# apapiu/transformer_latent_diffusion

Measured on AMD Instinct MI355X. Metric: images/sec (256px, 35-step CFG sampling), denoiser only, higher is better.
Workload: dtype bf16; 1 GPU; C1: 100M-param denoiser (d=768, L=12), 32x32x4 latents, 35 steps + CFG 6, DPM-Solver++(2M), 64 images/GPU (model batch 128); images_per_gpu=64, global_batch=64, n_iter=35, parallelism=single GPU

## Files before the change

transformer_latent_diffusion_amd/csrc/tld_gemm.hip:

```cpp
#include "../../include/tld_hip.h"
#include "tld_common.h"
#include "tld_attn_core.h"
#include <cstdlib>
#include <cstring>
#include <type_traits>

#ifdef TLD_DBG_EPI
#define TLD_EPI_BIT(b) ((p.dbg_epi & (b)) != 0)
#else
#define TLD_EPI_BIT(b) false
#endif

namespace tld {

namespace {

typedef const __attribute__((address_space(1))) void* gptr_t;
typedef __attribute__((address_space(3))) void* lptr_t;

__device__ __forceinline__ bf16x8 read_frag(const char* lds_tile, int row, int kchunk) {
    const int off = row * 128 + ((kchunk ^ ((row >> 1) & 7)) << 4);
    return *reinterpret_cast<const bf16x8*>(lds_tile + off);
}

// ... 30 lines not shown
    static constexpr int CB2_OFF = ROWSTAT2_OFF + 256 * 8;
    static constexpr int UPDW2_LDS = CB2_OFF + 2048;
    static constexpr int PLAINRS_OFF = LDS_BYTES;
    static constexpr int PLAINCB_OFF = PLAINRS_OFF + 256 * 8;
    static constexpr int PLAINLN_LDS = PLAINCB_OFF + 2048;
    static constexpr int SCRATCH = 4608;
    static constexpr int AT_K = STAGE_BYTES, AT_V = AT_K + 256 * 128, AT_Q = AT_V + 64 * kAttnVPitch, ATTN_LDS = AT_Q + 256 * 128;
};

template <int BN, int EPI, bool F8 = false, bool CONV = false, bool RING = false, bool TN = false>
__global__ __launch_bounds__(512) void gemm256p_kernel(GemmParams p, int nblocks) {
    using G = G256P<BN>;
    static_assert(!RING || BN == 256, "the half-tile ring exists for 256 x 256 tiles (bf16, and since round 6 MX-fp8)");
    static_assert(!TN || (BN == 256 && EPI == EPI_F32 && !F8 && !CONV && !RING), "transposed operands: fp32 output, 256 x 256 tiles, two-stage loop");
    using frag_t = std::conditional_t<F8, i32x8, bf16x8>;
    constexpr int ESZ = F8 ? 1 : 2;
    constexpr int SC_OFF = G::LDS_BYTES;
    static_assert(!F8 || (EPI == EPI_F32 || EPI == EPI_QKV || EPI == EPI_BIAS_BF16 || EPI == EPI_BIAS_RESID), "fp8 epilogues");
    static_assert(!CONV || (!F8 && (EPI == EPI_F32 || EPI == EPI_BIAS_BF16 || EPI == EPI_BIAS_RESID)), "conv mode");
    constexpr bool PLAIN_CB = EPI == EPI_BIAS_BF16 && BN != 384 && !F8 && !CONV;
    constexpr bool IS_QKV = EPI == EPI_QKV || EPI == EPI_QKV_LN, LN = EPI == EPI_QKV_LN || EPI == EPI_QKV_ATTN;
    constexpr bool UPDW = EPI == EPI_UP_DWCONV2 || EPI == EPI_UP_DWCONV32;
    static_assert(EPI != EPI_QKV_ATTN || (BN == 192 && !F8 && !CONV && !RING), "the fused attention epilogue is written for 256 x 192 tiles");
    static_assert(EPI != EPI_QKV_ATTN || G::ATTN_LDS <= 160 * 1024, "LDS");
    static_assert(8 * G::SCRATCH <= G::STAGE_BYTES, "epilogue scratch must fit in one stage");
    extern __shared__ __attribute__((aligned(16))) char smem[];
    const int lane = threadIdx.x & 63;
    const int wid = __builtin_amdgcn_readfirstlane(threadIdx.x >> 6);
    const int wm = wid / G::WN, wn = wid % G::WN;
    const int l31 = lane & 31, hi = lane >> 5;

    const int ntn = (p.N + BN - 1) / BN;
    const int ntm = (p.M + G::BM - 1) / G::BM;
    constexpr bool KSPLIT_OK = EPI == EPI_F32 && !F8 && !CONV && !RING && !TN;
    const int nsplit = (KSPLIT_OK && p.ksplit > 1) ? p.ksplit : 1;
    const int ntiles = ntm * ntn * nsplit;
    int kb_dec = 0;
    const int bid = blockIdx.x;
    const int xcd = bid & 7, lidx = bid >> 3;
    const int per_xcd_blocks = (nblocks + 7 - xcd) / 8;
    const int G2 = p.xcd_ngroups > 1 ? p.xcd_ngroups : 1;
    const int xn = xcd % G2, xm = xcd / G2, XM = 8 / G2;
    const int gcols = ntn / G2;
    const int r0 = (int)((long)ntm * xm / XM), r1 = (int)((long)ntm * (xm + 1) / XM);
    const int q = ntiles >> 3, rr = ntiles & 7;
    const int xbase = xcd < rr ? xcd * (q + 1) : rr * (q + 1) + (xcd - rr) * q;
    const int xcount = G2 > 1 ? (r1 - r0) * gcols : q + (xcd < rr ? 1 : 0);
    int my_tiles = lidx < xcount ? (xcount - lidx + per_xcd_blocks - 1) / per_xcd_blocks : 0;
    constexpr bool HT_OK = RING && !CONV && (EPI == EPI_F32 || EPI == EPI_QKV || EPI == EPI_QKV_LN || EPI == EPI_BIAS_BF16);
    const int ht_q = xcount / per_xcd_blocks, ht_R = xcount - ht_q * per_xcd_blocks;
    const bool ht = HT_OK && p.half_tail && G2 == 1 && ht_R > 0 && 2 * ht_R <= per_xcd_blocks;
    const int ht_qa = lidx >= ht_R ? 1 : 0;
    if (ht) my_tiles = ht_q + (lidx < 2 * ht_R ? 1 : 0);
// ... 4 lines not shown
    auto tile_coords = [&](int i, int& m0, int& n0) {
        const int t = item_tile(i);
        if (G2 > 1) {
            const int tm = t / gcols;
            m0 = (r0 + tm) * G::BM;
            n0 = (xn * gcols + (t - tm * gcols)) * BN;
        } else {
            int tile = xbase + t;
            if constexpr (KSPLIT_OK) {
                if (nsplit > 1) {
                    const int sp = tile / (ntm * ntn);
                    tile -= sp * (ntm * ntn);
                    kb_dec = sp * p.K * 2;
                }
            }
            const int tm = tile / ntn;
            m0 = tm * G::BM;
            n0 = (tile - tm * ntn) * BN;
        }
    };
    if (my_tiles == 0) return;

    const int nk = CONV ? 9 * (p.cv_cin >> 6) : p.K * ESZ / (G::BK * 2);
    unsigned voffA[G::A_PIECES], voffB[G::B_PIECES];
    unsigned cpix[G::A_PIECES], cbase[G::A_PIECES];
    size_t tnA = 0, tnW = 0;
    auto conv_tap = [&](int tap) {
        if constexpr (CONV) {
            const int ky = tap / 3;
            const int dy = ky - 1 + p.cv_down, dx = tap - ky * 3 - 1 + p.cv_down;
            const int ws_ = (p.cv_w >> p.cv_up) << p.cv_down;
            const unsigned sh = (unsigned)(p.cv_h << p.cv_down), sw = (unsigned)(p.cv_w << p.cv_down);
            int ln = lane;
            asm volatile("" : "+v"(ln));
#pragma unroll
            for (int q2 = 0; q2 < G::A_PIECES; ++q2) {
                const int r = (wid * G::A_PIECES + q2) * 8 + (ln >> 3);
                const unsigned c16 = (unsigned)(((ln & 7) ^ ((r >> 1) & 7)) * 16);
                const int yy = (int)(cpix[q2] >> 16) + dy, xx = (int)(cpix[q2] & 0xffffu) + dx;
                const bool inb = (unsigned)yy < sh && (unsigned)xx < sw;
                const unsigned sp = cbase[q2] + (unsigned)((yy >> p.cv_up) * ws_ + (xx >> p.cv_up));
                unsigned v = inb ? p.cv_data_off + sp * (unsigned)(p.cv_cin * 2) + c16 : c16;
                asm volatile("" : "+v"(v));
                voffA[q2] = v;
            }
        }
    };
// ... 28 lines not shown
                gr = gr < p.M ? gr : p.M - 1;
                const unsigned b = (unsigned)gr / hw, rem = (unsigned)gr - b * hw;
                const unsigned y = rem / (unsigned)p.cv_w, x = rem - y * (unsigned)p.cv_w;
                cpix[q2] = ((y << 16) | x) << p.cv_down;
                cbase[q2] = b * shw;
            }
            conv_tap(0);
        } else {
#pragma unroll
        for (int q2 = 0; q2 < G::A_PIECES; ++q2) {
            const int r = (wid * G::A_PIECES + q2) * 8 + (ln >> 3);
            const int clog = (ln & 7) ^ ((r >> 1) & 7);
            int gr = tm0 + r;
            gr = gr < p.M ? gr : p.M - 1;
            unsigned v = __umul24((unsigned)gr, (unsigned)(p.lda * ESZ)) + (unsigned)(clog * 16);
            asm volatile("" : "+v"(v));
            voffA[q2] = v;
        }
        }
        unsigned wgrp = 0;
        if constexpr (!F8 && !CONV && (EPI == EPI_F32 || EPI == EPI_BIAS_BF16)) {
            if (p.w_batch_rows) wgrp = (unsigned)(tm0 / p.w_batch_rows) * p.w_batch_stride_bytes;
        }
#pragma unroll
        for (int q2 = 0; q2 < G::B_PIECES; ++q2) {
            const int r = (wid * G::B_PIECES + q2) * 8 + (ln >> 3);
            const int clog = (ln & 7) ^ ((r >> 1) & 7);
            int gr = tn0 + r;
            gr = gr < p.N ? gr : p.N - 1;
            unsigned v = __umul24((unsigned)gr, (unsigned)(p.ldw * ESZ)) + (unsigned)(clog * 16) + wgrp;
            asm volatile("" : "+v"(v));
            voffB[q2] = v;
        }
    };
    int conv_akb = 0;
    auto dma_piece = [&](int q2, int kbyte, char* st) {
        if constexpr (TN) {
            const bool isA = q2 < G::A_PIECES;
            const char* base = isA ? reinterpret_cast<const char*>(p.A) + tnA + (size_t)(kbyte >> 7) * 64 * p.lda * 2
                                   : reinterpret_cast<const char*>(p.W) + tnW + (size_t)(kbyte >> 7) * 64 * p.ldw * 2;
            const unsigned vo = isA ? voffA[q2] : voffB[q2 - G::A_PIECES];
            __builtin_amdgcn_global_load_lds((gptr_t)(base + vo), (lptr_t)(st + (isA ? 0 : G::A_BYTES) + (wid * G::A_PIECES + (isA ? q2 : q2 - G::A_PIECES)) * 1024), 16, 0, 0);
            return;
        }
        if (q2 < G::A_PIECES) {
            const char* base = reinterpret_cast<const char*>(p.A) + (CONV ? conv_akb : kbyte);
            __builtin_amdgcn_global_load_lds((gptr_t)(base + voffA[q2]), (lptr_t)(st + (wid * G::A_PIECES + q2) * 1024), 16, 0, 0);
        } else {
            const char* base = reinterpret_cast<const char*>(p.W) + kbyte;
            __builtin_amdgcn_global_load_lds((gptr_t)(base + voffB[q2 - G::A_PIECES]),
                                             (lptr_t)(st + G::A_BYTES + (wid * G::B_PIECES + (q2 - G::A_PIECES)) * 1024), 16, 0, 0);
        }
    };
    auto dma_scales = [&](int tm0, int tn0, int kstep, int stage) {
        if constexpr (F8) {
            if (wid < 2) {
                const int rows = wid == 0 ? p.M : p.N;
                int r = (wid == 0 ? tm0 : tn0) + lane * 4;
                r = r + 3 < rows ? r : rows - 4;
                const uint8_t* src = (wid == 0 ? p.a_scale : p.w_scale) + ((size_t)kstep * rows + r) * 4;
                __builtin_amdgcn_global_load_lds((gptr_t)src, (lptr_t)(smem + SC_OFF + stage * 2048 + wid * 1024), 16, 0, 0);
            }
        }
    };
    auto issue = [&](int m0, int n0, int g) {
        char* st = smem + (g & 1) * G::STAGE_BYTES;
        set_offsets(m0, n0);
#pragma unroll
        for (int q2 = 0; q2 < G::A_PIECES + G::B_PIECES; ++q2) dma_piece(q2, KSPLIT_OK ? kb_dec : 0, st);
        dma_scales(m0, n0, 0, g & 1);
// ... 20 lines not shown
#pragma unroll
            for (int i = 0; i < G::TM; ++i) a[i] = rd(tnoA[i]);
#pragma unroll
            for (int j = 0; j < G::TN; ++j) b[j] = rd(tnoB[j]);
        } else if constexpr (!F8) {
            const int kc = ks * 2 + hi;
#pragma unroll
            for (int i = 0; i < G::TM; ++i) a[i] = read_frag(st, wm * G::WROWS + i * 32 + l31, kc);
#pragma unroll
            for (int j = 0; j < G::TN; ++j) b[j] = read_frag(st + G::A_BYTES, wn * G::WCOLS + j * 32 + l31, kc);
        } else {
            const int c = ks * 4 + hi;
            auto rd = [&](const char* base, int row) {
                const int sw = (row >> 1) & 7;
                const u32x4 lo = *reinterpret_cast<const u32x4*>(base + row * 128 + ((c ^ sw) << 4));
                const u32x4 hi4 = *reinterpret_cast<const u32x4*>(base + row * 128 + (((c + 2) ^ sw) << 4));
                return i32x8{(int)lo[0], (int)lo[1], (int)lo[2], (int)lo[3], (int)hi4[0], (int)hi4[1], (int)hi4[2], (int)hi4[3]};
            };
#pragma unroll
            for (int i = 0; i < G::TM; ++i) a[i] = rd(st, wm * G::WROWS + i * 32 + l31);
#pragma unroll
            for (int j = 0; j < G::TN; ++j) b[j] = rd(st + G::A_BYTES, wn * G::WCOLS + j * 32 + l31);
        }
    };

    constexpr int HT = 16384;
    unsigned rvA[RING ? 4 : 1], rvB[RING ? 4 : 1];
    unsigned rcpix[RING && CONV ? 4 : 1], rcbase[RING && CONV ? 4 : 1];
    int sc_m0 = 0, sc_n0 = 0;
    auto ring_conv_tap = [&](int tap) {
        if constexpr (RING && CONV) {
            const int ky = tap / 3;
            const int dy = ky - 1 + p.cv_down, dx = tap - ky * 3 - 1 + p.cv_down;
            const int ws_ = (p.cv_w >> p.cv_up) << p.cv_down;
            const unsigned sh = (unsigned)(p.cv_h << p.cv_down), sw = (unsigned)(p.cv_w << p.cv_down);
            unsigned full = ~0u;
            asm volatile("" : "+s"(full));
            int ln = (int)__builtin_amdgcn_mbcnt_hi(full, __builtin_amdgcn_mbcnt_lo(full, 0u));
            asm volatile("" : "+v"(ln));
#pragma unroll
            for (int h = 0; h < 2; ++h)
#pragma unroll
                for (int q2 = 0; q2 < 2; ++q2) {
                    const int r = (wid * 2 + q2) * 8 + (ln >> 3);
                    const unsigned c16 = (unsigned)(((ln & 7) ^ ((r >> 1) & 7)) * 16);
                    const int yy = (int)(rcpix[h * 2 + q2] >> 16) + dy, xx = (int)(rcpix[h * 2 + q2] & 0xffffu) + dx;
// ... 91 lines not shown

    int m0, n0;
    tile_coords(0, m0, n0);
    int kb0 = kb_dec, kbn = 0;
    if constexpr (!RING) issue(m0, n0, 0);
    int g = 0;
    int ctap = 0, ccb = 0;
    const int kpt = CONV ? (p.cv_cin >> 6) : 1;
    for (int it = 0; it < my_tiles; ++it) {
        int m0n = 0, n0n = 0;
        const bool has_next = it + 1 < my_tiles;
        if (has_next) { tile_coords(it + 1, m0n, n0n); kbn = kb_dec; }
        constexpr bool swapped = EPI != EPI_F32 && !UPDW;
        bool v_tile = false;
        if constexpr (IS_QKV) v_tile = n0 >= 2 * p.d;

        int nkt = nk;
        if constexpr (TN) {
            const int split = p.w_batch_rows ? m0 / p.w_batch_rows : 0;
            const int rows = p.tn_ktotal - split * p.K;
            nkt = (rows < p.K ? rows : p.K) >> 6;
        }
        const bool hmode = ht && it == ht_q;
        f32x16 acc[G::TM][G::TN];
#pragma unroll
        for (int i = 0; i < G::TM; ++i)
#pragma unroll
            for (int j = 0; j < G::TN; ++j)
#pragma unroll
                for (int r = 0; r < 16; ++r) acc[i][j][r] = 0.f;

        frag_t a0[G::TM], b0[G::TN];
        int sca[G::TM], scb[G::TN];
        auto aux_dma = [&]() {
            if constexpr (LN) {
                static_assert(kLnSlots == 8, "one partial-sum row is 64 B");
#pragma unroll
                for (int q2 = 0; q2 < 2; ++q2) {
                    const int piece = wid * 2 + q2;
                    int row = m0 + piece * 16 + (lane >> 2);
                    row = row < p.M ? row : p.M - 1;
                    const char* src = reinterpret_cast<const char*>(p.ln_stats) + (size_t)row * 64 + (lane & 3) * 16;
                    __builtin_amdgcn_global_load_lds((gptr_t)src, (lptr_t)(smem + G::LN_RAW + piece * 1024), 16, 0, 0);
                }
                if (wid < 2) {
                    int col = n0 + lane * 4;
                    col = col < p.N ? col : 0;
                    const float* src = (wid == 0 ? p.ln_c1 : p.ln_b1) + col;
                    __builtin_amdgcn_global_load_lds((gptr_t)src, (lptr_t)(smem + G::LN_CB + wid * 1024), 16, 0, 0);
                }
            }
            if constexpr (EPI == EPI_BIAS_BF16) {
                if (BN != 384 && p.row_stats && wid < 2) {
                    int r0s = m0 + wid * 128 + lane * 2;
                    r0s = r0s + 1 < p.M ? r0s : (p.M >= 2 ? p.M - 2 : 0);
// ... 3 lines not shown
                if constexpr (PLAIN_CB) {
                    if (wid == 3 || (wid == 2 && p.row_stats)) {
                        int col = n0 + lane * 4;
                        col = col < p.N ? col : 0;
                        const float* src = (wid == 2 ? p.ln_c1 : p.bias) + col;
                        __builtin_amdgcn_global_load_lds((gptr_t)src, (lptr_t)(smem + G::PLAINCB_OFF + (wid - 2) * 1024), 16, 0, 0);
                    }
                }
            }
            if constexpr (UPDW) {
                constexpr int RS_OFF = G::ROWSTAT2_OFF;
                if (p.row_stats && wid < 2) {
                    const char* src = reinterpret_cast<const char*>(p.row_stats + m0) + wid * 1024 + lane * 16;
                    __builtin_amdgcn_global_load_lds((gptr_t)src, (lptr_t)(smem + RS_OFF + wid * 1024), 16, 0, 0);
                }
                if (wid == 3 || (wid == 2 && p.row_stats)) {
                    const float* src = (wid == 2 ? p.ln_c1 : p.bias) + n0 + lane * 4;
                    __builtin_amdgcn_global_load_lds((gptr_t)src, (lptr_t)(smem + G::CB2_OFF + (wid - 2) * 1024), 16, 0, 0);
                }
            }
        };
        auto kloop = [&](auto swp) {
            constexpr bool SW = decltype(swp)::value;
            auto mma = [&](const frag_t (&a)[G::TM], const frag_t (&b)[G::TN], auto slice) {
                constexpr int S2 = decltype(slice)::value * 2;
#pragma unroll
                for (int i = 0; i < G::TM; ++i)
#pragma unroll
                    for (int j = 0; j < G::TN; ++j) {
                        if constexpr (F8) {
                            if constexpr (SW) acc[i][j] = __builtin_amdgcn_mfma_scale_f32_32x32x64_f8f6f4(b[j], a[i], acc[i][j], 0, 0, S2, scb[j], S2, sca[i]);
                            else acc[i][j] = __builtin_amdgcn_mfma_scale_f32_32x32x64_f8f6f4(a[i], b[j], acc[i][j], 0, 0, S2, sca[i], S2, scb[j]);
                        } else {
                            if constexpr (SW) acc[i][j] = __builtin_amdgcn_mfma_f32_32x32x16_bf16(b[j], a[i], acc[i][j], 0, 0, 0);
                            else acc[i][j] = __builtin_amdgcn_mfma_f32_32x32x16_bf16(a[i], b[j], acc[i][j], 0, 0, 0);
                        }
                    }
            };
            constexpr int NP = G::A_PIECES + G::B_PIECES;
            {
            const int grp = wid >> 2;
            wait_vmcnt<0>();
            __builtin_amdgcn_s_barrier();
            if (grp) __builtin_amdgcn_s_barrier();
            for (int k = 0; k < nkt; ++k, ++g) {
                if (k == (nkt > 1 ? 1 : 0)) aux_dma();
                const char* st = smem + (g & 1) * G::STAGE_BYTES;
                char* nst = smem + ((g + 1) & 1) * G::STAGE_BYTES;
                const bool more = (k + 1 < nkt) || (has_next && !UPDW);
                const int pkb = (k + 1 < nkt) ? (KSPLIT_OK ? kb0 : 0) + (k + 1) * G::BK * 2 : (KSPLIT_OK ? kbn : 0);
                if constexpr (CONV) {
                    if (k + 1 < nkt) {
                        if (++ccb == kpt) { ccb = 0; ++ctap; conv_tap(ctap); }
                    } else { ccb = 0; ctap = 0; }
                    conv_akb = ccb * (G::BK * 2);
                }
                if (k + 1 == nkt && more) set_offsets(m0n, n0n);
                constexpr int NI = F8 ? 2 : 4;
                constexpr int NDMA = (NI == 4) ? 2 : 1;
#pragma unroll
                for (int h = 0; h < NI; ++h) {
                    load_frags(st, h, a0, b0);
                    if constexpr (F8) {
                        if (h == 0) {
                            const char* sc = smem + SC_OFF + (g & 1) * 2048;
#pragma unroll
                            for (int i = 0; i < G::TM; ++i) sca[i] = *reinterpret_cast<const int*>(sc + (wm * G::WROWS + i * 32 + l31) * 4) >> (8 * hi);
#pragma unroll
                            for (int j = 0; j < G::TN; ++j) scb[j] = *reinterpret_cast<const int*>(sc + 1024 + (wn * G::WCOLS + j * 32 + l31) * 4) >> (8 * hi);
                        }
                    }
                    if (h < NDMA && more) {
                        constexpr int PER = (NP + NDMA - 1) / NDMA;
#pragma unroll
                        for (int q2 = 0; q2 < NP; ++q2) {
                            if (q2 < h * PER || q2 >= (h + 1) * PER) continue;
                            dma_piece(q2, pkb, nst);
                        }
                        if (h == 0) {
                            if (k + 1 < nkt) dma_scales(m0, n0, k + 1, (g + 1) & 1);
                            else dma_scales(m0n, n0n, 0, (g + 1) & 1);
                        }
                    }
                    if (h == NI - 1) wait_vmcnt<0>();
                    if (h == NI - 1) asm volatile("s_waitcnt lgkmcnt(0)" ::: "memory");
                    __builtin_amdgcn_sched_barrier(0);
                    __builtin_amdgcn_s_barrier();
                    __builtin_amdgcn_sched_barrier(0);
                    __builtin_amdgcn_s_setprio(1);
                    if constexpr (F8) {
                        if (h == 0) mma(a0, b0, std::integral_constant<int, 0>{}); else mma(a0, b0, std::integral_constant<int, 1>{});
                    } else {
                        mma(a0, b0, std::integral_constant<int, 0>{});
                    }
                    __builtin_amdgcn_s_setprio(0);
                    if (h == NI - 1) wait_vmcnt<0>();
                    __builtin_amdgcn_sched_barrier(0);
                    __builtin_amdgcn_s_barrier();
                    __builtin_amdgcn_sched_barrier(0);
                }
            }
            if (!grp) __builtin_amdgcn_s_barrier();
            }
        };
        auto kloop_ring = [&](auto swp) {
            if constexpr (RING) {
            constexpr bool SW = decltype(swp)::value;
            constexpr bool NOXT = UPDW;
            using I0 = std::integral_constant<int, 0>; using I1 = std::integral_constant<int, 1>;
            using I2 = std::integral_constant<int, 2>; using I3 = std::integral_constant<int, 3>;
            const int grp = wid >> 2;
            const int nj = nk >> 1;
            const bool xt = has_next && !NOXT;
            constexpr int RW = F8 ? 7 : 6;
            if (it == 0 || NOXT) {
                aux_dma();
                ring_offsets(m0, n0);
                ring_stage(I0{}, 0, 0); ring_stage(I1{}, 0, 1); ring_stage(I2{}, 0, 2); ring_stage(I3{}, 0, 3);
                ring_stage(I0{}, 1, 4); ring_stage(I1{}, 1, 5); ring_stage(I2{}, 1, 6);
                wait_vmcnt<RW>();
                __builtin_amdgcn_s_barrier();
            } else {
                __builtin_amdgcn_s_barrier();
// ... 118 lines not shown
                    }
                    }
                    __builtin_amdgcn_sched_barrier(0);
                    __builtin_amdgcn_s_barrier();
                    __builtin_amdgcn_sched_barrier(0);
                };
                phase(std::integral_constant<int, 1>{}); phase(std::integral_constant<int, 2>{});
                phase(std::integral_constant<int, 3>{}); phase(std::integral_constant<int, 4>{});
                phase(std::integral_constant<int, 5>{}); phase(std::integral_constant<int, 6>{});
                phase(std::integral_constant<int, 7>{}); phase(std::integral_constant<int, 8>{});
            };
            for (int j = 0; j + 1 < nj; ++j) iter(j, std::false_type{});
            iter(nj - 1, std::true_type{});
            if (xt) wait_vmcnt<0>();
            if (!grp) __builtin_amdgcn_s_barrier();
            g += nk;
            }
        };
        if constexpr (RING) {
            if constexpr (swapped) kloop_ring(std::true_type{}); else kloop_ring(std::false_type{});
        } else {
            if constexpr (swapped) kloop(std::true_type{}); else kloop(std::false_type{});
        }

        const int row0 = m0 + wm * G::WROWS;
        const int col0 = n0 + wn * G::WCOLS;
        auto gn_combine = [&](const float2* red) {
            if constexpr (CONV) {
                asm volatile("s_waitcnt lgkmcnt(0)" ::: "memory");
                __builtin_amdgcn_s_barrier();
                const int tid = wid * 64 + lane;
                const int qpg = p.gn_cpg >> 2;
                if (tid < BN / p.gn_cpg) {
                    float a = 0.f, a2 = 0.f;
                    for (int w2 = 0; w2 < G::WMc; ++w2)
                        for (int k2 = 0; k2 < qpg; ++k2) { const float2 t = red[w2 * (BN / 4) + tid * qpg + k2]; a += t.x; a2 += t.y; }
                    const int bb = m0 / p.gn_hw;
                    const int chunk = (m0 - bb * p.gn_hw) >> 8, nchunk = p.gn_hw >> 8;
                    p.gn_partial[((size_t)bb * nchunk + chunk) * p.gn_groups + n0 / p.gn_cpg + tid] = make_float2(a, a2);
                }
            }
        };
        if constexpr (EPI == EPI_F32) {
#pragma unroll
            for (int i = 0; i < G::TM; ++i)
#pragma unroll
// ... 198 lines not shown
                            oo[0] = (bf16)o0[0]; oo[1] = (bf16)o0[1]; oo[2] = (bf16)o1[0]; oo[3] = (bf16)o1[1];
                            if (!TLD_EPI_BIT(1)) {
                                TLD_STORE(reinterpret_cast<bf16x4*>(dst0 + ((size_t)rr * 16 + 2 * q) * p.ldo), oe);
                                TLD_STORE(reinterpret_cast<bf16x4*>(dst0 + ((size_t)rr * 16 + 2 * q + 1) * p.ldo), oo);
                            }
                        }
                    };
                    u32x4 c0v[4], c1v[4], c2v[4];
                    zero(c0v);
                    ld(0, c1v);
#pragma unroll 1
                    for (int q = 0; q < 6; q += 3) {
                        ld(q + 1, c2v); emit(c0v, c1v, c2v, q);
                        ld(q + 2, c0v); emit(c1v, c2v, c0v, q + 1);
                        ld(q + 3, c1v); emit(c2v, c0v, c1v, q + 2);
                    }
                    ld(7, c2v); emit(c0v, c1v, c2v, 6);
                    zero(c0v); emit(c1v, c2v, c0v, 7);
                }
                __builtin_amdgcn_s_barrier();
                if constexpr (!RING) { if (has_next) issue(m0n, n0n, g); }
            } else if constexpr (EPI == EPI_BIAS_RESID) {
                constexpr int P = 32 * 4 + 16;
                float gsum[CONV ? G::TN : 1], gsq[CONV ? G::TN : 1];
                if constexpr (CONV) {
#pragma unroll
                    for (int j = 0; j < G::TN; ++j) { gsum[j] = 0.f; gsq[j] = 0.f; }
                }
                resid4_t rnx[4];
                auto rfetch1 = [&](int i2, int j2, int itr) {
                    const int idx = itr * 64 + lane;
                    const int row = row0 + i2 * 32 + (idx >> 3), col = col0 + j2 * 32 + (idx & 7) * 4;
                    if (row < p.M && col < p.N && !TLD_EPI_BIT(16)) rnx[itr] = rs_raw4(p.resid + (size_t)row * p.ldr + col);
                    else rnx[itr] = resid4_t{};
                };
#pragma unroll
                for (int itr = 0; itr < 4; ++itr) rfetch1(0, 0, itr);
#pragma unroll
                for (int i = 0; i < G::TM; ++i) {
                    float ps[4] = {0.f, 0.f, 0.f, 0.f}, pq[4] = {0.f, 0.f, 0.f, 0.f};
#pragma unroll
                    for (int j = 0; j < G::TN; ++j) {
#pragma unroll
                        for (int rq = 0; rq < 4; ++rq) {
                            const int cl = 8 * rq + 4 * hi;
                            const int cg = col0 + j * 32 + cl < p.N ? col0 + j * 32 + cl : 0;
                            const float4 bv = *reinterpret_cast<const float4*>(p.bias + cg);
                            float4 v;
                            v.x = acc[i][j][rq * 4 + 0] + bv.x; v.y = acc[i][j][rq * 4 + 1] + bv.y;
                            v.z = acc[i][j][rq * 4 + 2] + bv.z; v.w = acc[i][j][rq * 4 + 3] + bv.w;
                            *reinterpret_cast<float4*>(ws + l31 * P + cl * 4) = v;
                        }
#pragma unroll
                        for (int itr = 0; itr < 4; ++itr) {
                            const int idx = itr * 64 + lane;
                            const int rl = idx >> 3, ch = idx & 7;
                            const float4 v = *reinterpret_cast<const float4*>(ws + rl * P + ch * 16);
                            const int row = row0 + i * 32 + rl, col = col0 + j * 32 + ch * 4;
                            if (row < p.M && col < p.N) {
                                resid_t* px = p.resid + (size_t)row * p.ldr + col;
                                float4 o = rs_widen4(rnx[itr]);
                                o.x += v.x; o.y += v.y; o.z += v.z; o.w += v.w;
                                if (!TLD_EPI_BIT(1)) rs_store4(px, o);
                                if constexpr (CONV) {
                                    const float r0 = rs_round(o.x), r1 = rs_round(o.y), r2 = rs_round(o.z), r3 = rs_round(o.w);
                                    gsum[j] += (r0 + r1) + (r2 + r3);
                                    gsq[j] = fmaf(r0, r0, fmaf(r1, r1, fmaf(r2, r2, fmaf(r3, r3, gsq[j]))));
                                }
                                if constexpr (G::WCOLS == 96) {
                                    const float r0 = rs_round(o.x), r1 = rs_round(o.y), r2 = rs_round(o.z), r3 = rs_round(o.w);
                                    ps[itr] += (r0 + r1) + (r2 + r3);
                                    pq[itr] = fmaf(r0, r0, fmaf(r1, r1, fmaf(r2, r2, fmaf(r3, r3, pq[itr]))));
                                }
                            }
                            if (j + 1 < G::TN) rfetch1(i, j + 1, itr); else if (i + 1 < G::TM) rfetch1(i + 1, 0, itr);
                        }
                    }
                    if constexpr (G::WCOLS == 96) {
                        if (p.stats_out) {
                            const int slot = (n0 + wn * G::WCOLS) / 96;
#pragma unroll
                            for (int itr = 0; itr < 4; ++itr) {
                                float a = ps[itr], q2 = pq[itr];
                                a = dpp_add<0xB1>(a); q2 = dpp_add<0xB1>(q2);
                                a = dpp_add<0x4E>(a); q2 = dpp_add<0x4E>(q2);
                                a = dpp_add<0x141>(a); q2 = dpp_add<0x141>(q2);
                                const int row = row0 + i * 32 + itr * 8 + (lane >> 3);
                                if ((lane & 7) == 0 && row < p.M && slot < kLnSlots) p.stats_out[(size_t)row * kLnSlots + slot] = make_float2(a, q2);
                            }
                        }
                    }
                }
                if constexpr (CONV) {
                    if (p.gn_partial) {
                        float2* red = reinterpret_cast<float2*>(smem + ((g - 1) & 1) * G::STAGE_BYTES + 8 * G::SCRATCH);
#pragma unroll
                        for (int j = 0; j < G::TN; ++j) {
                            float a = gsum[j], a2 = gsq[j];
#pragma unroll
                            for (int o2 = 8; o2 < 64; o2 <<= 1) { a += __shfl_xor(a, o2, 64); a2 += __shfl_xor(a2, o2, 64); }
                            if (lane < 8) red[wm * (BN / 4) + wn * (G::WCOLS / 4) + j * 8 + lane] = make_float2(a, a2);
                        }
                        gn_combine(red);
                    }
                }
            } else if constexpr (EPI == EPI_QKV_ATTN) {
                int e_lane = lane, e_l31 = l31, e_hi = hi;
                asm volatile("" : "+v"(e_lane), "+v"(e_l31), "+v"(e_hi));
                {
                    const int tid = wid * 64 + e_lane;
                    const int s0 = (tid & 1) * 4;
// ... 466 lines not shown
```

transformer_latent_diffusion_amd/csrc/tld_gemm_params.h:

```cpp
#pragma once
#include <stdint.h>
#ifndef __HIP__
struct float2;
#endif

namespace tld {

typedef __bf16 bf16;

#ifdef TLD_RESID_FP32
typedef float resid_t;
#else
#define TLD_RESID_BF16 1
typedef __bf16 resid_t;
#endif

constexpr int kLnSlots = 8;

enum GemmEpilogue {
    EPI_F32 = 0,
    EPI_QKV = 1,
    EPI_BIAS_BF16 = 2,
    EPI_BIAS_RESID = 3,
    EPI_QKV_LN = 5,
    EPI_UP_DWCONV32 = 4,
    EPI_UP_DWCONV2 = 6,
    EPI_QKV_ATTN = 7,
};

struct GemmParams {
    const bf16* A; int lda;
    const bf16* W; int ldw;
    int M, N, K;
    float* c_f32; int ldc;
    bf16* out_bf16; int ldo;
    bf16* vt;
    int ntok, d;
// ... 30 lines not shown
```

transformer_latent_diffusion_amd/csrc/tld_updw.hip:

```cpp
#include "tld_common.h"
#include <cstdlib>
#include <type_traits>

namespace tld {

namespace {

typedef const __attribute__((address_space(1))) void* gptr_t;
typedef __attribute__((address_space(3))) void* lptr_t;

struct PP {
    static constexpr int A_SLOT = 16384, B_SLOT = 8192;
    static constexpr int A_RING = 0, B_RING = 3 * A_SLOT;
    static constexpr int RING_BYTES = 3 * (A_SLOT + B_SLOT);
    static constexpr int PITCH = 512, IMG_BYTES = 128 * PITCH;
    static constexpr int ZROW = RING_BYTES;
    static constexpr int RS = ZROW + 8 * PITCH;
    static constexpr int CB = RS + 256 * 8;
    static constexpr int LDS = CB + 1024;
};
static_assert(PP::IMG_BYTES <= PP::RING_BYTES, "the image overlays the ring");
static_assert(2 * PP::LDS <= 160 * 1024, "two workgroups per CU");

template <int N> __device__ __forceinline__ void pp_wait_vmcnt() {
// ... 347 lines not shown
                ld(q + 1, c2v); emit(c0v, c1v, c2v, q);
                ld(q + 2, c0v); emit(c1v, c2v, c0v, q + 1);
                ld(q + 3, c1v); emit(c2v, c0v, c1v, q + 2);
            }
            ld(7, c2v); emit(c0v, c1v, c2v, 6);
            zero(c0v); emit(c1v, c2v, c0v, 7);
        }
        }
        asm volatile("s_waitcnt lgkmcnt(0)" ::: "memory");
        __builtin_amdgcn_s_barrier();
    }
}


struct DP {
    static constexpr int A_BYTES = 128 * 128, B_BYTES = 192 * 128, KT_BYTES = A_BYTES + B_BYTES;
    static constexpr int LDS = 3 * KT_BYTES;
    static constexpr int SCRATCH = 4608;
};

template <int TM>
__global__ __launch_bounds__(256, 2) void down_pp_kernel(GemmParams p, int nblocks) {
    constexpr int BM = 64 * TM, NA = 2 * TM;
    extern __shared__ __attribute__((aligned(16))) char smem[];
    const int tid = threadIdx.x;
    const int lane = tid & 63;
    const int wid = __builtin_amdgcn_readfirstlane(tid >> 6);
    const int wm = wid >> 1, wn = wid & 1;
    const int ntn = p.N / 192, ntm = p.M / BM, ntiles = ntm * ntn;
    const int nk = p.K >> 6;
    const unsigned lda2 = (unsigned)p.lda * 2u, ldw2 = (unsigned)p.ldw * 2u;
    unsigned ra0, rb0;
    {
        int l31v = lane & 31, hiv = lane >> 5;
        asm volatile("" : "+v"(l31v), "+v"(hiv));
        const int sw = (l31v >> 1) & 7;
        ra0 = (unsigned)((wm * 32 * TM + l31v) * 128 + ((hiv ^ sw) << 4));
        rb0 = (unsigned)(DP::A_BYTES + (wn * 96 + l31v) * 128 + ((hiv ^ sw) << 4));
    }
    for (int tile = blockIdx.x; tile < ntiles; tile += nblocks) {
        const int tm = tile / ntn;
        const int m0 = tm * BM, n0 = (tile - tm * ntn) * 192;
        unsigned vA[2], vB[2];
        {
            int ln = lane;
            asm volatile("" : "+v"(ln));
#pragma unroll
            for (int o = 0; o < 2; ++o) {
                const int r = (wid * NA + o) * 8 + (ln >> 3);
                unsigned va = __umul24((unsigned)(m0 + r), lda2) + (unsigned)(((ln & 7) ^ ((r >> 1) & 7)) * 16);
                const int rb_ = (wid * 6 + o) * 8 + (ln >> 3);
                unsigned vb = __umul24((unsigned)(n0 + rb_), ldw2) + (unsigned)(((ln & 7) ^ ((rb_ >> 1) & 7)) * 16);
                asm volatile("" : "+v"(va), "+v"(vb));
                vA[o] = va; vB[o] = vb;
            }
        }
        auto stageA = [&](int t, int slot, int lo, int hi_) {
#pragma unroll
            for (int q2 = 0; q2 < NA; ++q2) {
                if (q2 < lo || q2 >= hi_) continue;
                const char* base = reinterpret_cast<const char*>(p.A) + (size_t)t * 128 + (size_t)((q2 >> 1) * 16) * lda2;
                asm volatile("" : "+s"(base));
                unsigned o = vA[q2 & 1];
                asm volatile("" : "+v"(o));
                __builtin_amdgcn_global_load_lds((gptr_t)(base + o), (lptr_t)(smem + slot * DP::KT_BYTES + (wid * NA + q2) * 1024), 16, 0, 0);
            }
        };
        auto stageB = [&](int t, int slot, int lo, int hi_) {
#pragma unroll
            for (int q2 = 0; q2 < 6; ++q2) {
                if (q2 < lo || q2 >= hi_) continue;
                const char* base = reinterpret_cast<const char*>(p.W) + (size_t)t * 128 + (size_t)((q2 >> 1) * 16) * ldw2;
                asm volatile("" : "+s"(base));
                unsigned o = vB[q2 & 1];
                asm volatile("" : "+v"(o));
                __builtin_amdgcn_global_load_lds((gptr_t)(base + o), (lptr_t)(smem + slot * DP::KT_BYTES + DP::A_BYTES + (wid * 6 + q2) * 1024), 16, 0, 0);
            }
        };
        f32x16 acc[TM][3];
#pragma unroll
        for (int i = 0; i < TM; ++i)
#pragma unroll
            for (int j = 0; j < 3; ++j)
#pragma unroll
                for (int r = 0; r < 16; ++r) acc[i][j][r] = 0.f;

        bf16x8 fa[2][TM][2], fb[2][3][2];
        auto read_frags = [&](auto bufc, int slot, int h) {
            constexpr int bf = decltype(bufc)::value;
            const unsigned base = (unsigned)(slot * DP::KT_BYTES);
            unsigned a = ra0, b = rb0;
            asm volatile("" : "+v"(a), "+v"(b));
#pragma unroll
            for (int kk = 0; kk < 2; ++kk) {
                const unsigned kx = (unsigned)((2 * h + kk) << 5);
#pragma unroll
                for (int i = 0; i < TM; ++i) fa[bf][i][kk] = *reinterpret_cast<const bf16x8*>(smem + ((a ^ kx) + base) + i * 4096);
#pragma unroll
                for (int j = 0; j < 3; ++j) fb[bf][j][kk] = *reinterpret_cast<const bf16x8*>(smem + ((b ^ kx) + base) + j * 4096);
            }
        };
        auto mma = [&](auto bufc, auto&& side) {
            constexpr int bf = decltype(bufc)::value;
#pragma unroll
            for (int kk = 0; kk < 2; ++kk)
#pragma unroll
                for (int i = 0; i < TM; ++i) {
#pragma unroll
                    for (int j = 0; j < 3; ++j)
                        acc[i][j] = __builtin_amdgcn_mfma_f32_32x32x16_bf16(fb[bf][j][kk], fa[bf][i][kk], acc[i][j], 0, 0, 0);
                    __builtin_amdgcn_sched_barrier(0);
                    side(kk * TM + i);
                    __builtin_amdgcn_sched_barrier(0);
                }
        };
        using B0 = std::integral_constant<int, 0>; using B1 = std::integral_constant<int, 1>;
        auto slot3 = [](int k) { return k - (k / 3) * 3; };

        stageA(0, 0, 0, NA); stageB(0, 0, 0, 6); stageA(1, 1, 0, NA); stageB(1, 1, 0, 6);
        pp_wait_vmcnt<0>();
        __builtin_amdgcn_s_barrier();
        read_frags(B0{}, 0, 0);
        asm volatile("s_waitcnt lgkmcnt(0)" ::: "memory");
        for (int t = 0; t < nk; ++t) {
            const int s0 = slot3(t), s1 = slot3(t + 1), s2 = slot3(t + 2);
            const bool st = t + 2 < nk;
// ... 19 lines not shown
            asm volatile("s_waitcnt lgkmcnt(0)" ::: "memory");
            __builtin_amdgcn_s_barrier();
        }

        int lanev = lane;
        asm volatile("" : "+v"(lanev));
        const int l31 = lanev & 31, hi = lanev >> 5;
        char* ws = smem + wid * DP::SCRATCH;
        const int row0 = m0 + wm * 32 * TM, col0 = n0 + wn * 96;
        constexpr int P = 32 * 4 + 16;
        resid4_t rnx[4];
        auto rfetch1 = [&](int i2, int j2, int itr) {
            const int idx = itr * 64 + lanev;
            const int row = row0 + i2 * 32 + (idx >> 3), col = col0 + j2 * 32 + (idx & 7) * 4;
            rnx[itr] = rs_raw4(p.resid + (size_t)row * p.ldr + col);
        };
#pragma unroll
        for (int itr = 0; itr < 4; ++itr) rfetch1(0, 0, itr);
#pragma unroll
        for (int i = 0; i < TM; ++i) {
            float ps[4] = {0.f, 0.f, 0.f, 0.f}, pq[4] = {0.f, 0.f, 0.f, 0.f};
#pragma unroll
            for (int j = 0; j < 3; ++j) {
#pragma unroll
                for (int rq = 0; rq < 4; ++rq) {
                    const int cl = 8 * rq + 4 * hi;
                    const float4 bv = *reinterpret_cast<const float4*>(p.bias + col0 + j * 32 + cl);
                    float4 v;
                    v.x = acc[i][j][rq * 4 + 0] + bv.x; v.y = acc[i][j][rq * 4 + 1] + bv.y;
                    v.z = acc[i][j][rq * 4 + 2] + bv.z; v.w = acc[i][j][rq * 4 + 3] + bv.w;
                    *reinterpret_cast<float4*>(ws + l31 * P + cl * 4) = v;
                }
#pragma unroll
                for (int itr = 0; itr < 4; ++itr) {
                    const int idx = itr * 64 + lanev;
                    const int rl = idx >> 3, ch = idx & 7;
                    const float4 v = *reinterpret_cast<const float4*>(ws + rl * P + ch * 16);
                    const int row = row0 + i * 32 + rl, col = col0 + j * 32 + ch * 4;
                    resid_t* px = p.resid + (size_t)row * p.ldr + col;
                    float4 o = rs_widen4(rnx[itr]);
                    o.x += v.x; o.y += v.y; o.z += v.z; o.w += v.w;
                    rs_store4(px, o);
                    const float r0 = rs_round(o.x), r1 = rs_round(o.y), r2 = rs_round(o.z), r3 = rs_round(o.w);
                    ps[itr] += (r0 + r1) + (r2 + r3);
                    pq[itr] = fmaf(r0, r0, fmaf(r1, r1, fmaf(r2, r2, fmaf(r3, r3, pq[itr]))));
                    if (j + 1 < 3) rfetch1(i, j + 1, itr); else if (i + 1 < TM) rfetch1(i + 1, 0, itr);
                }
            }
            if (p.stats_out) {
                const int slot = col0 / 96;
#pragma unroll
                for (int itr = 0; itr < 4; ++itr) {
                    float a = ps[itr], q2 = pq[itr];
                    a = dpp_add<0xB1>(a); q2 = dpp_add<0xB1>(q2);
// ... 42 lines not shown
```

Measured before the change: 303.4 images/s.

## Use 16x16x32 MFMA tiles for bias-residual down-projection GEMMs

```diff
diff --git a/transformer_latent_diffusion_amd/csrc/tld_gemm.hip b/transformer_latent_diffusion_amd/csrc/tld_gemm.hip
--- a/transformer_latent_diffusion_amd/csrc/tld_gemm.hip
+++ b/transformer_latent_diffusion_amd/csrc/tld_gemm.hip
@@ -76,6 +76,8 @@
     constexpr bool IS_QKV = EPI == EPI_QKV || EPI == EPI_QKV_LN, LN = EPI == EPI_QKV_LN || EPI == EPI_QKV_ATTN;
     constexpr bool UPDW = EPI == EPI_UP_DWCONV2 || EPI == EPI_UP_DWCONV32;
     static_assert(EPI != EPI_QKV_ATTN || (BN == 192 && !F8 && !CONV && !RING), "the fused attention epilogue is written for 256 x 192 tiles");
+    constexpr bool MF16 = TLD_DOWN_MFMA16 && EPI == EPI_BIAS_RESID && !F8 && !CONV && !RING && !TN && (BN == 384 || BN == 192);
+    constexpr int HA16 = G::WROWS / 32;
     static_assert(EPI != EPI_QKV_ATTN || G::ATTN_LDS <= 160 * 1024, "LDS");
     static_assert(8 * G::SCRATCH <= G::STAGE_BYTES, "epilogue scratch must fit in one stage");
     extern __shared__ __attribute__((aligned(16))) char smem[];
@@ -83,6 +85,7 @@
     const int wid = __builtin_amdgcn_readfirstlane(threadIdx.x >> 6);
     const int wm = wid / G::WN, wn = wid % G::WN;
     const int l31 = lane & 31, hi = lane >> 5;
+    const int l15 = lane & 15, q4 = lane >> 4;
 
     const int ntn = (p.N + BN - 1) / BN;
     const int ntm = (p.M + G::BM - 1) / G::BM;
@@ -133,7 +136,7 @@
     if (my_tiles == 0) return;
 
     const int nk = CONV ? 9 * (p.cv_cin >> 6) : p.K * ESZ / (G::BK * 2);
-    unsigned voffA[G::A_PIECES], voffB[G::B_PIECES];
+    unsigned voffA[G::A_PIECES], voffB[MF16 ? 2 : G::B_PIECES];
     unsigned cpix[G::A_PIECES], cbase[G::A_PIECES];
     size_t tnA = 0, tnW = 0;
     auto conv_tap = [&](int tap) {
@@ -208,6 +211,17 @@
         if constexpr (!F8 && !CONV && (EPI == EPI_F32 || EPI == EPI_BIAS_BF16)) {
             if (p.w_batch_rows) wgrp = (unsigned)(tm0 / p.w_batch_rows) * p.w_batch_stride_bytes;
         }
+        if constexpr (MF16) {
+#pragma unroll
+            for (int q2 = 0; q2 < 2; ++q2) {
+                const int r = (wid * G::B_PIECES + q2) * 8 + (ln >> 3);
+                const int clog = (ln & 7) ^ ((r >> 1) & 7);
+                unsigned v = __umul24((unsigned)(tn0 + r), (unsigned)(p.ldw * ESZ)) + (unsigned)(clog * 16);
+                asm volatile("" : "+v"(v));
+                voffB[q2] = v;
+            }
+            return;
+        }
 #pragma unroll
         for (int q2 = 0; q2 < G::B_PIECES; ++q2) {
             const int r = (wid * G::B_PIECES + q2) * 8 + (ln >> 3);
@@ -232,6 +246,10 @@
         if (q2 < G::A_PIECES) {
             const char* base = reinterpret_cast<const char*>(p.A) + (CONV ? conv_akb : kbyte);
             __builtin_amdgcn_global_load_lds((gptr_t)(base + voffA[q2]), (lptr_t)(st + (wid * G::A_PIECES + q2) * 1024), 16, 0, 0);
+        } else if constexpr (MF16) {
+            const int qb = q2 - G::A_PIECES;
+            const char* base = reinterpret_cast<const char*>(p.W) + kbyte + (size_t)((qb >> 1) * 16) * (size_t)(p.ldw * ESZ);
+            __builtin_amdgcn_global_load_lds((gptr_t)(base + voffB[qb & 1]), (lptr_t)(st + G::A_BYTES + (wid * G::B_PIECES + qb) * 1024), 16, 0, 0);
         } else {
             const char* base = reinterpret_cast<const char*>(p.W) + kbyte;
             __builtin_amdgcn_global_load_lds((gptr_t)(base + voffB[q2 - G::A_PIECES]),
@@ -298,6 +316,23 @@
 #pragma unroll
             for (int j = 0; j < G::TN; ++j) b[j] = rd(st + G::A_BYTES, wn * G::WCOLS + j * 32 + l31);
         }
+    };
+
+    unsigned ra16 = 0, rb16 = 0;
+    if constexpr (MF16) {
+        const unsigned c16 = (unsigned)((q4 ^ ((l15 >> 1) & 7)) << 4);
+        ra16 = (unsigned)((wm * G::WROWS + l15) * 128) + c16;
+        rb16 = (unsigned)(G::A_BYTES + (wn * G::WCOLS + l15) * 128) + c16;
+    }
+    auto load_frags16 = [&](const char* st, int ks, auto halfc, bf16x8 (&a)[HA16], bf16x8 (&b)[6]) {
+        constexpr int half = decltype(halfc)::value;
+        const unsigned kx = (unsigned)(ks << 6);
+        if constexpr (half == 0) {
+#pragma unroll
+            for (int j = 0; j < 6; ++j) b[j] = *reinterpret_cast<const bf16x8*>(st + (rb16 ^ kx) + j * 2048);
+        }
+#pragma unroll
+        for (int i = 0; i < HA16; ++i) a[i] = *reinterpret_cast<const bf16x8*>(st + (ra16 ^ kx) + (half * HA16 + i) * 2048);
     };
 
     constexpr int HT = 16384;
@@ -435,15 +470,24 @@
             nkt = (rows < p.K ? rows : p.K) >> 6;
         }
         const bool hmode = ht && it == ht_q;
-        f32x16 acc[G::TM][G::TN];
+        f32x16 acc[MF16 ? 1 : G::TM][MF16 ? 1 : G::TN];
+        f32x4 acc16[MF16 ? 2 * HA16 : 1][MF16 ? 6 : 1];
+        if constexpr (MF16) {
+#pragma unroll
+            for (int i = 0; i < 2 * HA16; ++i)
+#pragma unroll
+                for (int j = 0; j < 6; ++j) acc16[i][j] = f32x4{0.f, 0.f, 0.f, 0.f};
+        } else {
 #pragma unroll
         for (int i = 0; i < G::TM; ++i)
 #pragma unroll
             for (int j = 0; j < G::TN; ++j)
 #pragma unroll
                 for (int r = 0; r < 16; ++r) acc[i][j][r] = 0.f;
-
-        frag_t a0[G::TM], b0[G::TN];
+        }
+
+        frag_t a0[MF16 ? 1 : G::TM], b0[MF16 ? 1 : G::TN];
+        bf16x8 a16[HA16], b16[6];
         int sca[G::TM], scb[G::TN];
         auto aux_dma = [&]() {
             if constexpr (LN) {
@@ -493,7 +537,15 @@
         };
         auto kloop = [&](auto swp) {
             constexpr bool SW = decltype(swp)::value;
-            auto mma = [&](const frag_t (&a)[G::TM], const frag_t (&b)[G::TN], auto slice) {
+            auto mma16 = [&](auto halfc) {
+                constexpr int half = decltype(halfc)::value;
+#pragma unroll
+                for (int i = 0; i < HA16; ++i)
+#pragma unroll
+                    for (int j = 0; j < 6; ++j)
+                        acc16[half * HA16 + i][j] = __builtin_amdgcn_mfma_f32_16x16x32_bf16(b16[j], a16[i], acc16[half * HA16 + i][j], 0, 0, 0);
+            };
+            auto mma = [&](const frag_t (&a)[MF16 ? 1 : G::TM], const frag_t (&b)[MF16 ? 1 : G::TN], auto slice) {
                 constexpr int S2 = decltype(slice)::value * 2;
 #pragma unroll
                 for (int i = 0; i < G::TM; ++i)
@@ -514,7 +566,7 @@
             wait_vmcnt<0>();
             __builtin_amdgcn_s_barrier();
             if (grp) __builtin_amdgcn_s_barrier();
-            for (int k = 0; k < nkt; ++k, ++g) {
+            auto kstep = [&](int k) {
                 if (k == (nkt > 1 ? 1 : 0)) aux_dma();
                 const char* st = smem + (g & 1) * G::STAGE_BYTES;
                 char* nst = smem + ((g + 1) & 1) * G::STAGE_BYTES;
@@ -531,7 +583,12 @@
                 constexpr int NDMA = (NI == 4) ? 2 : 1;
 #pragma unroll
                 for (int h = 0; h < NI; ++h) {
-                    load_frags(st, h, a0, b0);
+                    if constexpr (MF16) {
+                        if (h & 1) load_frags16(st, h >> 1, std::integral_constant<int, 1>{}, a16, b16);
+                        else load_frags16(st, h >> 1, std::integral_constant<int, 0>{}, a16, b16);
+                    } else {
+                        load_frags(st, h, a0, b0);
+                    }
                     if constexpr (F8) {
                         if (h == 0) {
                             const char* sc = smem + SC_OFF + (g & 1) * 2048;
@@ -559,7 +616,9 @@
                     __builtin_amdgcn_s_barrier();
                     __builtin_amdgcn_sched_barrier(0);
                     __builtin_amdgcn_s_setprio(1);
-                    if constexpr (F8) {
+                    if constexpr (MF16) {
+                        if (h & 1) mma16(std::integral_constant<int, 1>{}); else mma16(std::integral_constant<int, 0>{});
+                    } else if constexpr (F8) {
                         if (h == 0) mma(a0, b0, std::integral_constant<int, 0>{}); else mma(a0, b0, std::integral_constant<int, 1>{});
                     } else {
                         mma(a0, b0, std::integral_constant<int, 0>{});
@@ -570,6 +629,12 @@
                     __builtin_amdgcn_s_barrier();
                     __builtin_amdgcn_sched_barrier(0);
                 }
+            };
+            if constexpr (MF16) {
+#pragma clang loop unroll(disable)
+                for (int k = 0; k < nkt; ++k, ++g) kstep(k);
+            } else {
+                for (int k = 0; k < nkt; ++k, ++g) kstep(k);
             }
             if (!grp) __builtin_amdgcn_s_barrier();
             }
@@ -734,6 +799,7 @@
         } else {
             if constexpr (swapped) kloop(std::true_type{}); else kloop(std::false_type{});
         }
+        if constexpr (MF16) __builtin_amdgcn_sched_barrier(0);
 
         const int row0 = m0 + wm * G::WROWS;
         const int col0 = n0 + wn * G::WCOLS;
@@ -978,6 +1044,9 @@
                 if constexpr (!RING) { if (has_next) issue(m0n, n0n, g); }
             } else if constexpr (EPI == EPI_BIAS_RESID) {
                 constexpr int P = 32 * 4 + 16;
+                int elane = lane;
+                if constexpr (MF16) asm volatile("" : "+v"(elane));
+                const int e_l15 = elane & 15, e_q4 = elane >> 4;
                 float gsum[CONV ? G::TN : 1], gsq[CONV ? G::TN : 1];
                 if constexpr (CONV) {
 #pragma unroll
@@ -985,7 +1054,7 @@
                 }
                 resid4_t rnx[4];
                 auto rfetch1 = [&](int i2, int j2, int itr) {
-                    const int idx = itr * 64 + lane;
+                    const int idx = itr * 64 + elane;
                     const int row = row0 + i2 * 32 + (idx >> 3), col = col0 + j2 * 32 + (idx & 7) * 4;
                     if (row < p.M && col < p.N && !TLD_EPI_BIT(16)) rnx[itr] = rs_raw4(p.resid + (size_t)row * p.ldr + col);
                     else rnx[itr] = resid4_t{};
@@ -995,8 +1064,22 @@
 #pragma unroll
                 for (int i = 0; i < G::TM; ++i) {
                     float ps[4] = {0.f, 0.f, 0.f, 0.f}, pq[4] = {0.f, 0.f, 0.f, 0.f};
+                    int q4i = e_q4;
+                    if constexpr (MF16) asm volatile("" : "+v"(q4i));
 #pragma unroll
                     for (int j = 0; j < G::TN; ++j) {
+                        if constexpr (MF16) {
+#pragma unroll
+                            for (int ii = 0; ii < 2; ++ii)
+#pragma unroll
+                                for (int jj = 0; jj < 2; ++jj) {
+                                    const int cl = 16 * jj + 4 * q4i;
+                                    const int cg = col0 + j * 32 + cl < p.N ? col0 + j * 32 + cl : 0;
+                                    const float4 bv = *reinterpret_cast<const float4*>(p.bias + cg);
+                                    const f32x4 c = acc16[2 * i + ii][2 * j + jj];
+                                    *reinterpret_cast<float4*>(ws + (16 * ii + e_l15) * P + cl * 4) = make_float4(c[0] + bv.x, c[1] + bv.y, c[2] + bv.z, c[3] + bv.w);
+                                }
+                        } else {
 #pragma unroll
                         for (int rq = 0; rq < 4; ++rq) {
                             const int cl = 8 * rq + 4 * hi;
@@ -1007,9 +1090,10 @@
                             v.z = acc[i][j][rq * 4 + 2] + bv.z; v.w = acc[i][j][rq * 4 + 3] + bv.w;
                             *reinterpret_cast<float4*>(ws + l31 * P + cl * 4) = v;
                         }
+                        }
 #pragma unroll
                         for (int itr = 0; itr < 4; ++itr) {
-                            const int idx = itr * 64 + lane;
+                            const int idx = itr * 64 + elane;
                             const int rl = idx >> 3, ch = idx & 7;
                             const float4 v = *reinterpret_cast<const float4*>(ws + rl * P + ch * 16);
                             const int row = row0 + i * 32 + rl, col = col0 + j * 32 + ch * 4;
@@ -1041,8 +1125,8 @@
                                 a = dpp_add<0xB1>(a); q2 = dpp_add<0xB1>(q2);
                                 a = dpp_add<0x4E>(a); q2 = dpp_add<0x4E>(q2);
                                 a = dpp_add<0x141>(a); q2 = dpp_add<0x141>(q2);
-                                const int row = row0 + i * 32 + itr * 8 + (lane >> 3);
-                                if ((lane & 7) == 0 && row < p.M && slot < kLnSlots) p.stats_out[(size_t)row * kLnSlots + slot] = make_float2(a, q2);
+                                const int row = row0 + i * 32 + itr * 8 + (elane >> 3);
+                                if ((elane & 7) == 0 && row < p.M && slot < kLnSlots) p.stats_out[(size_t)row * kLnSlots + slot] = make_float2(a, q2);
                             }
                         }
                     }
diff --git a/transformer_latent_diffusion_amd/csrc/tld_gemm_params.h b/transformer_latent_diffusion_amd/csrc/tld_gemm_params.h
--- a/transformer_latent_diffusion_amd/csrc/tld_gemm_params.h
+++ b/transformer_latent_diffusion_amd/csrc/tld_gemm_params.h
@@ -13,6 +13,10 @@
 #else
 #define TLD_RESID_BF16 1
 typedef __bf16 resid_t;
+#endif
+
+#ifndef TLD_DOWN_MFMA16
+#define TLD_DOWN_MFMA16 1
 #endif
 
 constexpr int kLnSlots = 8;
diff --git a/transformer_latent_diffusion_amd/csrc/tld_updw.hip b/transformer_latent_diffusion_amd/csrc/tld_updw.hip
--- a/transformer_latent_diffusion_amd/csrc/tld_updw.hip
+++ b/transformer_latent_diffusion_amd/csrc/tld_updw.hip
@@ -393,6 +393,7 @@
 template <int TM>
 __global__ __launch_bounds__(256, 2) void down_pp_kernel(GemmParams p, int nblocks) {
     constexpr int BM = 64 * TM, NA = 2 * TM;
+    constexpr bool MF16 = TLD_DOWN_MFMA16 != 0;
     extern __shared__ __attribute__((aligned(16))) char smem[];
     const int tid = threadIdx.x;
     const int lane = tid & 63;
@@ -403,7 +404,7 @@
     const unsigned lda2 = (unsigned)p.lda * 2u, ldw2 = (unsigned)p.ldw * 2u;
     unsigned ra0, rb0;
     {
-        int l31v = lane & 31, hiv = lane >> 5;
+        int l31v = MF16 ? lane & 15 : lane & 31, hiv = MF16 ? lane >> 4 : lane >> 5;
         asm volatile("" : "+v"(l31v), "+v"(hiv));
         const int sw = (l31v >> 1) & 7;
         ra0 = (unsigned)((wm * 32 * TM + l31v) * 128 + ((hiv ^ sw) << 4));
@@ -448,13 +449,21 @@
                 __builtin_amdgcn_global_load_lds((gptr_t)(base + o), (lptr_t)(smem + slot * DP::KT_BYTES + DP::A_BYTES + (wid * 6 + q2) * 1024), 16, 0, 0);
             }
         };
-        f32x16 acc[TM][3];
+        f32x16 acc[MF16 ? 1 : TM][MF16 ? 1 : 3];
+        f32x4 acc16[MF16 ? 2 * TM : 1][MF16 ? 6 : 1];
+        if constexpr (MF16) {
+#pragma unroll
+            for (int i = 0; i < 2 * TM; ++i)
+#pragma unroll
+                for (int j = 0; j < 6; ++j) acc16[i][j] = f32x4{0.f, 0.f, 0.f, 0.f};
+        } else {
 #pragma unroll
         for (int i = 0; i < TM; ++i)
 #pragma unroll
             for (int j = 0; j < 3; ++j)
 #pragma unroll
                 for (int r = 0; r < 16; ++r) acc[i][j][r] = 0.f;
+        }
 
         bf16x8 fa[2][TM][2], fb[2][3][2];
         auto read_frags = [&](auto bufc, int slot, int h) {
@@ -462,6 +471,14 @@
             const unsigned base = (unsigned)(slot * DP::KT_BYTES);
             unsigned a = ra0, b = rb0;
             asm volatile("" : "+v"(a), "+v"(b));
+            if constexpr (MF16) {
+                const unsigned kx = (unsigned)(h << 6);
+#pragma unroll
+                for (int i = 0; i < 2 * TM; ++i) fa[bf][i >> 1][i & 1] = *reinterpret_cast<const bf16x8*>(smem + ((a ^ kx) + base) + i * 2048);
+#pragma unroll
+                for (int j = 0; j < 6; ++j) fb[bf][j >> 1][j & 1] = *reinterpret_cast<const bf16x8*>(smem + ((b ^ kx) + base) + j * 2048);
+                return;
+            }
 #pragma unroll
             for (int kk = 0; kk < 2; ++kk) {
                 const unsigned kx = (unsigned)((2 * h + kk) << 5);
@@ -473,6 +490,18 @@
         };
         auto mma = [&](auto bufc, auto&& side) {
             constexpr int bf = decltype(bufc)::value;
+            if constexpr (MF16) {
+#pragma unroll
+                for (int i = 0; i < 2 * TM; ++i) {
+#pragma unroll
+                    for (int j = 0; j < 6; ++j)
+                        acc16[i][j] = __builtin_amdgcn_mfma_f32_16x16x32_bf16(fb[bf][j >> 1][j & 1], fa[bf][i >> 1][i & 1], acc16[i][j], 0, 0, 0);
+                    __builtin_amdgcn_sched_barrier(0);
+                    side(i);
+                    __builtin_amdgcn_sched_barrier(0);
+                }
+                return;
+            }
 #pragma unroll
             for (int kk = 0; kk < 2; ++kk)
 #pragma unroll
@@ -538,6 +567,18 @@
             float ps[4] = {0.f, 0.f, 0.f, 0.f}, pq[4] = {0.f, 0.f, 0.f, 0.f};
 #pragma unroll
             for (int j = 0; j < 3; ++j) {
+                if constexpr (MF16) {
+                    const int l15 = lanev & 15, q4 = lanev >> 4;
+#pragma unroll
+                    for (int ii = 0; ii < 2; ++ii)
+#pragma unroll
+                        for (int jj = 0; jj < 2; ++jj) {
+                            const int cl = 16 * jj + 4 * q4;
+                            const float4 bv = *reinterpret_cast<const float4*>(p.bias + col0 + j * 32 + cl);
+                            const f32x4 c = acc16[2 * i + ii][2 * j + jj];
+                            *reinterpret_cast<float4*>(ws + (16 * ii + l15) * P + cl * 4) = make_float4(c[0] + bv.x, c[1] + bv.y, c[2] + bv.z, c[3] + bv.w);
+                        }
+                } else {
 #pragma unroll
                 for (int rq = 0; rq < 4; ++rq) {
                     const int cl = 8 * rq + 4 * hi;
@@ -546,6 +587,7 @@
                     v.x = acc[i][j][rq * 4 + 0] + bv.x; v.y = acc[i][j][rq * 4 + 1] + bv.y;
                     v.z = acc[i][j][rq * 4 + 2] + bv.z; v.w = acc[i][j][rq * 4 + 3] + bv.w;
                     *reinterpret_cast<float4*>(ws + l31 * P + cl * 4) = v;
+                }
                 }
 #pragma unroll
                 for (int itr = 0; itr < 4; ++itr) {
```

Result: no change. 305.1 images/s, median of 6 (+0.6%).
